# Y-Claw/Multilevel-GNN

Measured on AMD Instinct MI355X. Metric: graphs/sec fwd+bwd, 3-level GNN on 10k-node d=128 synthetic; HBM GB/s %peak, higher is better.
Workload: dtype f32; 1 GPU; configs[1]: ER graphs N=10000 E=160000 x64 per GPU, d=128, 3 GENConv(softmax, res+, LayerNorm) + projection pooling G=25000 k=2 + DiffPool 146->37->10, fp32; step = CSR build (of the next batch, on a second stream) + fwd + bwd + grad all-reduce + Adam; graphs_per_gpu=64, global_batch=64, parallelism=dp1, world_size=1, allreduce_bytes=1429768

## Files before the change

include/mlgnn.h:

```cpp
#ifndef MLGNN_H
#define MLGNN_H

#include <stdint.h>

#ifdef __cplusplus
extern "C" {
#endif

#define MLGNN_ABI_VERSION 19

#define MLGNN_E_NULL      (-1)
#define MLGNN_E_SHAPE     (-2)
#define MLGNN_E_MODE      (-3)
#define MLGNN_E_DTYPE     (-4)
#define MLGNN_E_WORKSPACE (-5)
#define MLGNN_E_ALIGN     (-6)

#define MLGNN_MSG_IDENTITY 0
#define MLGNN_MSG_WEIGHTED 1
#define MLGNN_MSG_GEN      2

#define MLGNN_EDGE_NONE  0
#define MLGNN_EDGE_RANK1 1
#define MLGNN_EDGE_FULL  2
// ... 105 lines not shown
                            float* workspace,
                            int64_t workspace_floats, const uint8_t* keep_mask, float keep_scale,
                            int64_t rows, int64_t d, int relu,
                            int dtype, void* stream);

int64_t mlgnn_linear_wgrad_workspace_floats(int64_t N, int64_t M, int64_t K, int dtype);
int mlgnn_linear_wgrad(const void* grad_out, const void* x, const float* x_gamma, const float* x_beta,
                       const float* grad_out_row_max, const float* x_row_max, float* grad_w_b, float* workspace,
                       int64_t workspace_floats, int64_t N, int64_t M, int64_t K, int dtype,
                       void* stream);

int mlgnn_diffpool_fwd_supported(int64_t N, int64_t K, int64_t C);
int mlgnn_diffpool_fwd(const void* z, const void* adj, const void* s_logits, void* s_out,
                       void* x_out, void* adj_out, float* partial, int64_t B, int64_t N,
                       int64_t K, int64_t C, int adj_batched, int dtype, void* stream);

int mlgnn_diffpool_bwd(const void* z, const void* adj, const void* s_softmax, const void* grad_x,
                       const void* grad_adj_out, const float* coef, void* grad_z, void* grad_s,
                       void* grad_adj, int64_t B, int64_t N, int64_t K, int64_t C,
                       int adj_batched, int dtype, void* stream);

int mlgnn_dense_sage_supported(int64_t n, int64_t C, int64_t O, int need_grad_adj);
int64_t mlgnn_dense_sage_bwd_workspace_floats(int64_t B, int64_t C, int64_t O);
int mlgnn_dense_sage_fwd(const void* x, const void* adj, const void* w_rel, const void* w_root,
                         const float* bias, void* y, float* rinv, int64_t B, int64_t n, int64_t C,
                         int64_t O, int adj_batched, int normalize, int dtype, void* stream);
int mlgnn_dense_sage_bwd(const void* grad_y, const void* y, const float* rinv, const void* x,
                         const void* adj, const void* w_rel, const void* w_root, void* grad_x,
                         void* grad_adj, float* grad_w, float* workspace, int64_t workspace_floats,
                         int64_t B, int64_t n, int64_t C, int64_t O, int adj_batched, int normalize,
                         int dtype, void* stream);

int64_t mlgnn_coo_to_csr_workspace_bytes(int64_t N, int64_t E);
int mlgnn_coo_to_csr(const int64_t* edge_index, int64_t E, int64_t N,
                     int32_t* rowptr, int32_t* col, int32_t* eid,
                     int32_t* rowptr_t, int32_t* col_t, int32_t* pos_t, int32_t* eid_t,
                     int32_t* bad_ids, void* workspace, int64_t workspace_bytes, void* stream);

int mlgnn_edge_table_to_csr(const float* attr, int64_t row_stride, int64_t r, int64_t width,
                            const int32_t* eid, const int32_t* eid_t, float* by_dst, float* by_src,
                            int64_t E, void* stream);

int64_t mlgnn_msgnorm_bwd_workspace_floats(int64_t rows, int64_t d);
int mlgnn_msgnorm_add_fwd(const void* x, const void* m, const float* scale, void* h,
                          int64_t rows, int64_t d, int dtype, void* stream);
int mlgnn_msgnorm_add_bwd(const void* grad_h, const void* x, const void* m, const float* scale,
                          void* grad_x, void* grad_m, float* grad_scale, float* workspace,
                          int64_t workspace_floats, int64_t rows, int64_t d, int dtype, void* stream);

int64_t mlgnn_segment_pool_workspace_bytes(int64_t B, int64_t d);
int mlgnn_segment_pool_fwd(const void* x, const int32_t* ptr, void* out, int32_t* argmax,
                           void* workspace, int64_t workspace_bytes, int64_t B, int64_t d,
                           int kind, int dtype, void* stream);

int mlgnn_tallgemm_supported(int64_t N, int64_t R, int64_t J, int dtype);
int64_t mlgnn_tallgemm_workspace_bytes(int64_t R, int64_t J, int dtype);
int mlgnn_tallgemm_nt(const void* a, const void* bt, int bt_transposed, const float* bias, const void* residual,
                      const float* row_max, int ln_mode, const float* gamma, const float* beta, float ln_eps,
                      float* rstd_out, float* row_max_out, void* c, void* workspace, int64_t workspace_bytes, int64_t N, int64_t R, int64_t J, int dtype, void* stream);

int mlgnn_tallgemm_nt_shift_supported(int64_t N, int64_t R, int64_t J);
int mlgnn_tallgemm_nt_shift(const float* a, const float* bt, int bt_transposed, const float* row_max, const float* lse,
                            const int32_t* rowptr, float* c, float* grad_shifted, int32_t* shift_flag, void* workspace,
                            int64_t workspace_bytes, int64_t N, int64_t R, int64_t J, void* stream);

int mlgnn_tallgemm_bf16_shift_supported(int64_t N, int64_t R, int64_t J);
// ... 232 lines not shown
```

multilevel-gnn_amd/csrc/graph.hip:

```cpp
#include <hipcub/hipcub.hpp>
#include "common.h"
#include "launch.h"
#include "mlgnn.h"

namespace mlgnn {

__device__ __forceinline__ int checked_id(int64_t v, int N, int* bad) {
  if (v < 0 || v >= N) {
    if (bad) atomicAdd(bad, 1);
    return v < 0 ? 0 : N - 1;
  }
  return (int)v;
}

constexpr int kCsrThreads = 1024, kCsrMaxPer = 20;
constexpr int kCsrWindow = 16384;
constexpr int kCsrTargetBlocks = 512;

__device__ __forceinline__ int csr_chunk_of_block() {
  const int nb = gridDim.x, q = nb / kXcds, r = nb % kXcds, xcd = blockIdx.x % kXcds;
  return (xcd < r ? xcd * (q + 1) : r * (q + 1) + (xcd - r) * q) + blockIdx.x / kXcds;
}

__device__ __forceinline__ int block_min(int v, int* slot) {
  if (threadIdx.x == 0) *slot = INT32_MAX;
  __syncthreads();
#pragma unroll
  for (int off = 32; off > 0; off >>= 1) v = min(v, __shfl_xor(v, off));
  if ((threadIdx.x & (kWave - 1)) == 0) atomicMin(slot, v);
  __syncthreads();
  return *slot;
}

__device__ __forceinline__ void csr_count_side(const int64_t* __restrict__ in64, int* __restrict__ out32,
                                               int* __restrict__ cnt, int64_t e0, int64_t n, int per, int N, int* bad,
                                               int* h, int* slot) {
  int k[kCsrMaxPer];
  int mk = INT32_MAX;
  const int64_t first = e0 + threadIdx.x;
  const int64_t left = n - first;
  const int lim = (int)(left < (int64_t)per * kCsrThreads ? (left < 0 ? 0 : left) : (int64_t)per * kCsrThreads);
  const int64_t* __restrict__ in = in64 + first;
  int* __restrict__ out = out32 + first;
#pragma unroll
  for (int g = 0; g < kCsrMaxPer; g += 5) {
    int64_t raw[5];
#pragma unroll
    for (int q = 0; q < 5; ++q) raw[q] = ((g + q) * kCsrThreads < lim) ? in[(g + q) * kCsrThreads] : -1;
#pragma unroll
    for (int q = 0; q < 5; ++q) {
      k[g + q] = -1;
      if ((g + q) * kCsrThreads < lim) {
        k[g + q] = checked_id(raw[q], N, bad);
        out[(g + q) * kCsrThreads] = k[g + q];
        mk = min(mk, k[g + q]);
      }
    }
    __builtin_amdgcn_sched_barrier(0);
  }
  for (int i = threadIdx.x; i < kCsrWindow / 4; i += kCsrThreads) reinterpret_cast<int4*>(h)[i] = make_int4(0, 0, 0, 0);
  const int base = block_min(mk, slot);
#pragma unroll
  for (int q = 0; q < kCsrMaxPer; ++q) {
    if (q >= per || k[q] < 0) continue;
    const int o = k[q] - base;
    if (o < kCsrWindow) atomicAdd(h + o, 1); else atomicAdd(cnt + k[q], 1);
  }
  __syncthreads();
  for (int i = threadIdx.x; i < kCsrWindow; i += kCsrThreads)
    if (h[i]) atomicAdd(cnt + base + i, h[i]);
  __syncthreads();
}

__global__ __launch_bounds__(kCsrThreads, 8) void csr_count_kernel(const int64_t* __restrict__ src64,
                                                                   const int64_t* __restrict__ dst64,
                                                                   int* __restrict__ src32, int* __restrict__ dst32,
                                                                   int* __restrict__ cnt_dst, int* __restrict__ cnt_src,
                                                                   int64_t n, int per, int N, int* bad) {
  __shared__ __attribute__((aligned(16))) int h[kCsrWindow];
  __shared__ int slot;
  const int64_t e0 = (int64_t)csr_chunk_of_block() * per * kCsrThreads;
  csr_count_side(dst64, dst32, cnt_dst, e0, n, per, N, bad, h, &slot);
  csr_count_side(src64, src32, cnt_src, e0, n, per, N, bad, h, &slot);
}

__global__ __launch_bounds__(kCsrThreads, 8) void csr_place_kernel(const int* __restrict__ key,
                                                                   const int* __restrict__ rowptr,
                                                                   int* __restrict__ cursor, int* __restrict__ out,
                                                                   int64_t n, int per) {
  __shared__ __attribute__((aligned(16))) int h[kCsrWindow];
  __shared__ int slot;
  const int64_t e0 = (int64_t)csr_chunk_of_block() * per * kCsrThreads;
  int k[kCsrMaxPer];
  int mk = INT32_MAX;
#pragma unroll
  for (int q = 0; q < kCsrMaxPer; ++q) {
    const int64_t i = e0 + threadIdx.x + (int64_t)q * kCsrThreads;
    k[q] = (q < per && i < n) ? key[i] : -1;
    if (k[q] >= 0) mk = min(mk, k[q]);
  }
  for (int i = threadIdx.x; i < kCsrWindow / 4; i += kCsrThreads) reinterpret_cast<int4*>(h)[i] = make_int4(0, 0, 0, 0);
  const int base = block_min(mk, &slot);
#pragma unroll
  for (int q = 0; q < kCsrMaxPer; ++q)
    if (q < per && k[q] >= 0 && k[q] - base < kCsrWindow) atomicAdd(h + (k[q] - base), 1);
  __syncthreads();
  for (int i = threadIdx.x; i < kCsrWindow; i += kCsrThreads) {
    const int c = h[i];
    if (c) h[i] = rowptr[base + i] + atomicAdd(cursor + base + i, c);
  }
  __syncthreads();
#pragma unroll
  for (int q = 0; q < kCsrMaxPer; ++q) {
    if (q >= per || k[q] < 0) continue;
    const int64_t i = e0 + threadIdx.x + (int64_t)q * kCsrThreads;
    const int o = k[q] - base;
    const int where = o < kCsrWindow ? atomicAdd(h + o, 1) : rowptr[k[q]] + atomicAdd(cursor + k[q], 1);
    out[where] = (int)i;
  }
}

template <int WIDTH>
__device__ __forceinline__ int wave_sort(int v, int lane) {
#pragma unroll
  for (int k = 2; k <= WIDTH; k <<= 1) {
    int p = lane ^ (k - 1);
    int o = __shfl(v, p);
    v = (lane < p) ? min(v, o) : max(v, o);
#pragma unroll
    for (int j = k >> 2; j >= 1; j >>= 1) {
      p = lane ^ j;
      o = __shfl(v, p);
      v = (lane < p) ? min(v, o) : max(v, o);
    }
  }
  return v;
}

struct RowOut { const int* src32; int* col; int* rowkey; const int* eid; int* col_t; int* eid_t; };

template <bool BY_SRC>
__device__ __forceinline__ void emit(const RowOut& o, int slot, int v, int row) {
  if constexpr (!BY_SRC) { o.col[slot] = o.src32[v]; o.rowkey[slot] = row; }
  else { o.col_t[slot] = o.rowkey[v]; o.eid_t[slot] = o.eid[v]; }
}

constexpr int kSortPairs = 4;
constexpr int kSortRows = 2 * kSortPairs;

template <bool BY_SRC>
__global__ __launch_bounds__(kBlock) void csr_sort_rows_kernel(const int* __restrict__ rowptr, int* __restrict__ data,
                                                               int N, int* __restrict__ long_rows,
                                                               int* __restrict__ long_count, const RowOut o) {
  const int lane = threadIdx.x & (kWave - 1);
  const int r0 = (blockIdx.x * kWavesPerBlock + threadIdx.x / kWave) * kSortRows;
  if (r0 >= N) return;
  const int rp = rowptr[min(r0 + min(lane, kSortRows), N)];
  const int deg_l = __shfl_down(rp, 1) - rp;
  const bool small = __builtin_amdgcn_ballot_w64(lane < kSortRows && deg_l > 32) == 0;
  if (small) {
    const int half = lane >> 5, l = lane & 31;
    int v[kSortPairs], beg[kSortPairs], dg[kSortPairs];
#pragma unroll
    for (int p = 0; p < kSortPairs; ++p) {
      beg[p] = __shfl(rp, 2 * p + half);
      dg[p] = __shfl(rp, 2 * p + half + 1) - beg[p];
      v[p] = l < dg[p] ? data[beg[p] + l] : INT32_MAX;
    }
#pragma unroll
    for (int p = 0; p < kSortPairs; ++p) v[p] = wave_sort<32>(v[p], lane);
    int g0[kSortPairs], g1[kSortPairs];
#pragma unroll
    for (int p = 0; p < kSortPairs; ++p) {
      g0[p] = 0; g1[p] = 0;
      if (l < dg[p]) {
        if constexpr (!BY_SRC) g0[p] = o.src32[v[p]];
        else { g0[p] = o.rowkey[v[p]]; g1[p] = o.eid[v[p]]; }
      }
    }
#pragma unroll
    for (int p = 0; p < kSortPairs; ++p) {
      if (l >= dg[p]) continue;
      const int slot = beg[p] + l;
      data[slot] = v[p];
      if constexpr (!BY_SRC) { o.col[slot] = g0[p]; o.rowkey[slot] = r0 + 2 * p + half; }
      else { o.col_t[slot] = g0[p]; o.eid_t[slot] = g1[p]; }
    }
    return;
  }
  for (int w = 0; w < kSortRows && r0 + w < N; ++w) {
    const int beg = __shfl(rp, w), deg = __shfl(rp, w + 1) - beg;
    if (deg <= kWave) {
      int v = lane < deg ? data[beg + lane] : INT32_MAX;
      v = wave_sort<kWave>(v, lane);
      if (lane < deg) { data[beg + lane] = v; emit<BY_SRC>(o, beg + lane, v, r0 + w); }
    } else if (lane == 0) {
      long_rows[atomicAdd(long_count, 1)] = r0 + w;
    }
  }
}

constexpr int kLongLds = 4096;
template <bool BY_SRC>
__global__ __launch_bounds__(kBlock) void csr_sort_long_rows_kernel(const int* __restrict__ rowptr,
                                                                    int* __restrict__ data,
                                                                    const int* __restrict__ long_rows,
                                                                    const int* __restrict__ long_count,
                                                                    const RowOut o) {
  __shared__ int buf[kLongLds];
  const int count = *long_count;
  for (int it = blockIdx.x; it < count; it += gridDim.x) {
    const int r = long_rows[it];
    const int beg = rowptr[r], n = rowptr[r + 1] - beg;
    int P = 1;
    while (P < n) P <<= 1;
    const bool in_lds = n <= kLongLds;
    int* a = in_lds ? buf : data + beg;
    if (in_lds) {
      for (int i = threadIdx.x; i < n; i += kBlock) buf[i] = data[beg + i];
    }
    __syncthreads();
    for (int k = 2; k <= P; k <<= 1) {
      for (int i = threadIdx.x; i < P / 2; i += kBlock) {
        const int blk = i / (k / 2), off = i % (k / 2);
        const int x = blk * k + off, y = blk * k + k - 1 - off;
        if (y < n) { const int u = a[x], w = a[y]; if (u > w) { a[x] = w; a[y] = u; } }
      }
      __syncthreads();
      for (int j = k >> 2; j >= 1; j >>= 1) {
        for (int i = threadIdx.x; i < P / 2; i += kBlock) {
          const int x = (i / j) * 2 * j + i % j, y = x + j;
// ... 16 lines not shown
                                  float* __restrict__ by_dst, float* __restrict__ by_src, int64_t n) {
  const int64_t i = (int64_t)blockIdx.x * blockDim.x + threadIdx.x;
  if (i >= n) return;
  const float* a = attr + (int64_t)eid[i] * stride;
  const float* b = attr + (int64_t)eid_t[i] * stride;
  for (int k = 0; k < width; ++k) {
    by_dst[i * width + k] = k < r ? a[k] : 0.f;
    by_src[i * width + k] = k < r ? b[k] : 0.f;
  }
}

__global__ __launch_bounds__(256) void edge_table_w1_kernel(const float* __restrict__ attr, int64_t stride,
                                                            const int4* __restrict__ eid, const int4* __restrict__ eid_t,
                                                            float4* __restrict__ by_dst, float4* __restrict__ by_src,
                                                            int64_t n4) {
  const int64_t i = (int64_t)blockIdx.x * blockDim.x + threadIdx.x;
  if (i >= n4) return;
  const int4 e = eid[i], t = eid_t[i];
  float4 a, b;
  a.x = attr[(int64_t)e.x * stride]; a.y = attr[(int64_t)e.y * stride];
  a.z = attr[(int64_t)e.z * stride]; a.w = attr[(int64_t)e.w * stride];
  b.x = attr[(int64_t)t.x * stride]; b.y = attr[(int64_t)t.y * stride];
  b.z = attr[(int64_t)t.z * stride]; b.w = attr[(int64_t)t.w * stride];
  by_dst[i] = a;
  by_src[i] = b;
}

static size_t scan_temp_bytes(int64_t n) {
  size_t bytes = 0;
  (void)hipcub::DeviceScan::ExclusiveSum(nullptr, bytes, (const int*)nullptr, (int*)nullptr, (int)n, (hipStream_t)0);
  return bytes;
}

struct CsrWs {
  int *src32, *dst32, *rowkey, *cnt_dst, *cnt_src, *cur_dst, *cur_src, *long_rows, *long_rows_t, *long_count;
  size_t zero_bytes;
  void* scan_temp; size_t scan_bytes; size_t total;
};
static CsrWs csr_ws(void* workspace, int64_t N, int64_t E) {
  CsrWs w;
  const size_t e4 = align256((size_t)E * 4), n4 = align256((size_t)(N + 1) * 4);
  char* p = (char*)(((uintptr_t)workspace + 255) & ~(uintptr_t)255);
  w.src32 = (int*)p; p += e4;
  w.dst32 = (int*)p; p += e4;
  w.rowkey = (int*)p; p += e4;
  w.long_rows = (int*)p; p += n4;
  w.long_rows_t = (int*)p; p += n4;
  w.cnt_dst = (int*)p; p += n4;
  w.cnt_src = (int*)p; p += n4;
  w.cur_dst = (int*)p; p += n4;
  w.cur_src = (int*)p; p += n4;
  w.long_count = (int*)p; p += 256;
  w.zero_bytes = (size_t)(p - (char*)w.cnt_dst);
  w.scan_bytes = scan_temp_bytes(N + 1);
  w.scan_temp = p; p += align256(w.scan_bytes);
  w.total = (size_t)(p - (char*)(((uintptr_t)workspace + 255) & ~(uintptr_t)255)) + 256;
  return w;
}

static int csr_per_thread(int64_t E) {
  const int64_t target = (E + kCsrTargetBlocks - 1) / kCsrTargetBlocks;
  const int64_t per = (target + kCsrThreads - 1) / kCsrThreads;
  return (int)(per < 1 ? 1 : per > kCsrMaxPer ? kCsrMaxPer : per);
}

}

using namespace mlgnn;

extern "C" int64_t mlgnn_coo_to_csr_workspace_bytes(int64_t N, int64_t E) {
  if (N < 0 || E < 0 || N > INT32_MAX - 1 || E > INT32_MAX) return MLGNN_E_SHAPE;
  return (int64_t)csr_ws(nullptr, N, E).total;
}

extern "C" int mlgnn_coo_to_csr(const int64_t* edge_index, int64_t E, int64_t N,
                                int32_t* rowptr, int32_t* col, int32_t* eid,
                                int32_t* rowptr_t, int32_t* col_t, int32_t* pos_t, int32_t* eid_t,
                                int32_t* bad_ids, void* workspace, int64_t workspace_bytes, void* stream) {
  if (N < 0 || E < 0 || N > INT32_MAX - 1 || E > INT32_MAX) return MLGNN_E_SHAPE;
  if (!rowptr || !rowptr_t) return MLGNN_E_NULL;
  hipStream_t s = (hipStream_t)stream;
  if (bad_ids) (void)hipMemsetAsync(bad_ids, 0, 4, s);
  if (E == 0) {
    (void)hipMemsetAsync(rowptr, 0, (size_t)(N + 1) * 4, s);
    (void)hipMemsetAsync(rowptr_t, 0, (size_t)(N + 1) * 4, s);
    return (int)hipGetLastError();
  }
  if (!edge_index || !col || !eid || !col_t || !pos_t || !eid_t || !workspace) return MLGNN_E_NULL;
  if (N == 0) return MLGNN_E_SHAPE;
  const CsrWs w = csr_ws(workspace, N, E);
  if (workspace_bytes < (int64_t)w.total) return MLGNN_E_WORKSPACE;
  const int per = csr_per_thread(E);
  const int64_t chunk = (int64_t)per * kCsrThreads;
  const unsigned gC = (unsigned)((E + chunk - 1) / chunk);
  const unsigned gRows = (unsigned)(((N + kSortRows - 1) / kSortRows + kWavesPerBlock - 1) / kWavesPerBlock);
  hipError_t err;

  (void)hipMemsetAsync(w.cnt_dst, 0, w.zero_bytes, s);
  hipLaunchKernelGGL(csr_count_kernel, dim3(gC), dim3(kCsrThreads), 0, s, edge_index, edge_index + E, w.src32,
                     w.dst32, w.cnt_dst, w.cnt_src, E, per, (int)N, bad_ids);
  size_t sb = w.scan_bytes;
  err = hipcub::DeviceScan::ExclusiveSum(w.scan_temp, sb, w.cnt_dst, rowptr, (int)(N + 1), s);
  if (err != hipSuccess) return (int)err;
  err = hipcub::DeviceScan::ExclusiveSum(w.scan_temp, sb, w.cnt_src, rowptr_t, (int)(N + 1), s);
  if (err != hipSuccess) return (int)err;

  RowOut o;
  o.src32 = w.src32; o.col = col; o.rowkey = w.rowkey; o.eid = eid; o.col_t = col_t; o.eid_t = eid_t;
  hipLaunchKernelGGL(csr_place_kernel, dim3(gC), dim3(kCsrThreads), 0, s, w.dst32, rowptr, w.cur_dst, eid, E, per);
  hipLaunchKernelGGL(csr_sort_rows_kernel<false>, dim3(gRows), dim3(kBlock), 0, s, rowptr, eid, (int)N, w.long_rows,
                     w.long_count, o);
  hipLaunchKernelGGL(csr_sort_long_rows_kernel<false>, dim3(256), dim3(kBlock), 0, s, rowptr, eid, w.long_rows,
                     w.long_count, o);

  hipLaunchKernelGGL(csr_place_kernel, dim3(gC), dim3(kCsrThreads), 0, s, col, rowptr_t, w.cur_src, pos_t, E, per);
  hipLaunchKernelGGL(csr_sort_rows_kernel<true>, dim3(gRows), dim3(kBlock), 0, s, rowptr_t, pos_t, (int)N, w.long_rows_t,
                     w.long_count + 1, o);
  hipLaunchKernelGGL(csr_sort_long_rows_kernel<true>, dim3(256), dim3(kBlock), 0, s, rowptr_t, pos_t, w.long_rows_t,
                     w.long_count + 1, o);
  return (int)hipGetLastError();
}

namespace mlgnn {
__global__ __launch_bounds__(256) void sage_rewrite_kernel(const int64_t* __restrict__ src, const int64_t* __restrict__ dst,
                                                          const float* __restrict__ attr, int64_t attr_stride,
                                                          int64_t* __restrict__ out_src, int64_t* __restrict__ out_dst,
                                                          float* __restrict__ out_w, int64_t E, int64_t N) {
  const int64_t stride = (int64_t)gridDim.x * blockDim.x;
  for (int64_t i = (int64_t)blockIdx.x * blockDim.x + threadIdx.x; i < E + N; i += stride) {
    if (i < E) {
      const int64_t a = src[i], b = dst[i];
      const bool loop = a == b;
      out_src[i] = loop ? N : a;
      out_dst[i] = loop ? N : b;
      if (out_w) out_w[i] = attr ? attr[i * attr_stride] : 1.f;
    } else {
      out_src[i] = i - E;
      out_dst[i] = i - E;
      if (out_w) out_w[i] = 1.f;
    }
  }
}
}

extern "C" int mlgnn_sage_rewrite(const int64_t* edge_index, const float* edge_attr, int64_t attr_stride, int64_t E,
                                  int64_t N, int64_t* out_edge_index, float* out_weight, void* stream) {
  if (N < 0 || E < 0 || N > INT32_MAX - 2 || E + N > INT32_MAX || (edge_attr && attr_stride < 1)) return MLGNN_E_SHAPE;
  if (E + N == 0) return 0;
  if ((E > 0 && !edge_index) || !out_edge_index) return MLGNN_E_NULL;
  const int64_t n = E + N;
// ... 76 lines not shown
```

multilevel-gnn_amd/mlgnn/_lib.py:

```python
import ctypes
import os

LIB = os.environ.get("MLGNN_LIB") or os.path.join(os.path.dirname(os.path.abspath(__file__)), "libmlgnn.so")

_c = ctypes
_P = _c.c_void_p
_I64 = _c.c_int64
_INT = _c.c_int
_F = _c.c_float

SIGNATURES = {
    "mlgnn_version": (_INT, []),
    "mlgnn_csr_aggregate_bwd_workspace_floats": (_I64, [_I64, _I64, _INT, _INT, _INT, _INT]),
    "mlgnn_csr_aggregate_fwd": (_INT, [_P, _P, _P, _P, _P, _P, _P, _P, _P, _P, _P, _P, _P,
                                       _I64, _I64, _INT, _INT, _INT, _INT, _INT, _F, _F, _P, _P, _F, _INT, _P, _P]),
    "mlgnn_csr_aggregate_bwd": (_INT, [_P, _P, _P, _P, _P, _P, _P, _P, _P, _P, _P, _P, _P, _P, _P,
                                       _P, _P, _P, _P, _I64,
                                       _I64, _I64, _INT, _INT, _INT, _INT, _INT, _INT, _F, _F, _P, _P, _F, _INT, _INT, _P,
                                       _P, _P, _P]),
    "mlgnn_csr_aggregate_bwd_ln_workspace_floats": (_I64, [_I64, _I64]),
    "mlgnn_csr_aggregate_bwd_ln": (_INT, [_P, _P, _P, _P, _P, _P, _P, _P, _P, _P, _P, _P, _P, _P, _P,
                                          _P, _P, _P, _P, _I64,
                                          _I64, _I64, _INT, _INT, _INT, _INT, _INT, _INT, _F, _F, _P, _P, _F, _INT, _INT, _P,
                                          _P, _P, _P, _P]),
# ... 1 lines not shown
    "mlgnn_power_bwd_prologue": (_INT, [_P, _P, _P, _P, _P, _F, _P, _P, _P, _P, _I64, _I64, _I64, _INT, _P]),
    "mlgnn_embedding_bwd": (_INT, [_P, _P, _P, _P, _I64, _I64, _INT, _P]),
    "mlgnn_max_table_grad_supported": (_INT, [_I64, _I64, _I64]),
    "mlgnn_max_table_grad_workspace_floats": (_I64, [_I64, _I64, _I64]),
    "mlgnn_max_table_grad": (_INT, [_P, _P, _P, _P, _P, _I64, _I64, _I64, _I64, _INT, _P]),
    "mlgnn_max_table_grad_by_type": (_INT, [_P, _P, _P, _P, _P, _P, _P, _P, _I64, _I64, _I64, _INT, _P]),
    "mlgnn_csr_aggregate_bwd_slots_offset_floats": (_I64, [_I64, _I64, _INT]),
    "mlgnn_max_sparse_supported": (_INT, [_I64, _I64]),
    "mlgnn_max_sparse_records": (_I64, [_I64, _I64, _I64]),
    "mlgnn_max_winners": (_INT, [_P, _P, _P, _P, _P, _I64, _I64, _P]),
    "mlgnn_max_sparse_bwd": (_INT, [_P, _P, _P, _P, _P, _P, _I64, _I64, _P]),
    "mlgnn_max_sparse_table_grad": (_INT, [_P, _P, _P, _P, _P, _I64, _I64, _I64, _INT, _P]),
    "mlgnn_table_grad_bytes": (_I64, [_I64, _I64]),
    "mlgnn_table_grad_begin": (_INT, [_P, _I64, _I64, _P, _P]),
    "mlgnn_table_grad_finish": (_INT, [_P, _P, _I64, _I64, _INT, _P]),
    "mlgnn_segment_project_fwd": (_INT, [_P, _P, _P, _P, _P, _P, _I64, _I64, _I64, _I64, _I64, _I64, _INT, _P]),
    "mlgnn_segment_project_bwd": (_INT, [_P, _P, _P, _P, _P, _P, _P, _P, _P, _P, _P,
                                         _I64, _I64, _I64, _I64, _I64, _I64, _I64, _INT, _P]),
    "mlgnn_layernorm_bwd_workspace_floats": (_I64, [_I64, _I64, _INT]),
    "mlgnn_layernorm_act_fwd": (_INT, [_P, _P, _P, _P, _P, _P, _P, _P, _F, _I64, _I64, _F, _INT, _INT, _P]),
    "mlgnn_layernorm_act_bwd": (_INT, [_P, _P, _P, _P, _P, _P, _P, _P, _P, _P, _P, _I64, _P, _F, _I64, _I64, _INT, _INT, _P]),
    "mlgnn_linear_wgrad_workspace_floats": (_I64, [_I64, _I64, _I64, _INT]),
    "mlgnn_tallgemm_bf16_shift_supported": (_INT, [_I64, _I64, _I64]),
    "mlgnn_tallgemm_bf16_shift": (_INT, [_P, _P, _P, _P, _P, _P, _P, _I64, _I64, _I64, _I64, _P]),
    "mlgnn_linear_bwd_supported": (_INT, [_I64, _I64, _I64, _INT]),
    "mlgnn_linear_bwd_workspace_floats": (_I64, [_I64, _I64, _I64, _INT]),
    "mlgnn_linear_bwd": (_INT, [_P, _P, _P, _P, _INT, _P, _INT, _P, _P, _P, _P, _P, _P, _P, _P, _P, _P, _I64,
                                _I64, _I64, _I64, _P]),
    "mlgnn_linear_wgrad": (_INT, [_P, _P, _P, _P, _P, _P, _P, _P, _I64, _I64, _I64, _I64, _INT, _P]),
    "mlgnn_diffpool_fwd_supported": (_INT, [_I64, _I64, _I64]),
    "mlgnn_diffpool_fwd": (_INT, [_P, _P, _P, _P, _P, _P, _P, _I64, _I64, _I64, _I64, _INT, _INT, _P]),
    "mlgnn_coo_to_csr_workspace_bytes": (_I64, [_I64, _I64]),
    "mlgnn_coo_to_csr": (_INT, [_P, _I64, _I64, _P, _P, _P, _P, _P, _P, _P, _P, _P, _I64, _P]),
    "mlgnn_msgnorm_bwd_workspace_floats": (_I64, [_I64, _I64]),
    "mlgnn_msgnorm_add_fwd": (_INT, [_P, _P, _P, _P, _I64, _I64, _INT, _P]),
    "mlgnn_msgnorm_add_bwd": (_INT, [_P, _P, _P, _P, _P, _P, _P, _P, _I64, _I64, _I64, _INT, _P]),
    "mlgnn_diffpool_bwd": (_INT, [_P, _P, _P, _P, _P, _P, _P, _P, _P, _I64, _I64, _I64, _I64, _INT, _INT, _P]),
    "mlgnn_edge_table_to_csr": (_INT, [_P, _I64, _I64, _I64, _P, _P, _P, _P, _I64, _P]),
    "mlgnn_dense_sage_supported": (_INT, [_I64, _I64, _I64, _INT]),
    "mlgnn_dense_sage_bwd_workspace_floats": (_I64, [_I64, _I64, _I64]),
    "mlgnn_dense_sage_fwd": (_INT, [_P, _P, _P, _P, _P, _P, _P, _I64, _I64, _I64, _I64, _INT, _INT, _INT, _P]),
    "mlgnn_dense_sage_bwd": (_INT, [_P, _P, _P, _P, _P, _P, _P, _P, _P, _P, _P, _I64,
                                    _I64, _I64, _I64, _I64, _INT, _INT, _INT, _P]),
    "mlgnn_segment_pool_workspace_bytes": (_I64, [_I64, _I64]),
    "mlgnn_segment_pool_fwd": (_INT, [_P, _P, _P, _P, _P, _I64, _I64, _I64, _INT, _INT, _P]),
    "mlgnn_tallgemm_supported": (_INT, [_I64, _I64, _I64, _INT]),
    "mlgnn_tallgemm_workspace_bytes": (_I64, [_I64, _I64, _INT]),
    "mlgnn_tallgemm_nt": (_INT, [_P, _P, _INT, _P, _P, _P, _INT, _P, _P, _F, _P, _P, _P, _P, _I64, _I64, _I64, _I64, _INT, _P]),
    "mlgnn_tallgemm_nt_shift_supported": (_INT, [_I64, _I64, _I64]),
    "mlgnn_tallgemm_nt_shift": (_INT, [_P, _P, _INT, _P, _P, _P, _P, _P, _P, _P, _I64, _I64, _I64, _I64, _P]),
    "mlgnn_tallgemm_lnin_postln_supported": (_INT, [_I64, _I64, _I64]),
    "mlgnn_tallgemm_lnin_postln": (_INT, [_P, _P, _P, _P, _P, _P, _P, _P, _P, _F, _INT, _P, _P, _P, _P, _P, _I64,
                                          _I64, _I64, _I64, _P]),
    "mlgnn_tallgemm_lnbwd_supported": (_INT, [_I64, _I64, _I64]),
    "mlgnn_tallgemm_lnbwd_workspace_bytes": (_I64, [_I64, _I64]),
    "mlgnn_tallgemm_lnbwd": (_INT, [_P, _P, _INT, _P, _P, _P, _P, _P, _P, _P, _P, _P, _I64, _I64, _I64, _I64, _P]),
    "mlgnn_csr_replicate": (_INT, [_P] * 14 + [_I64, _I64, _I64, _P]),
    "mlgnn_sage_rewrite": (_INT, [_P, _P, _I64, _I64, _I64, _P, _P, _P]),
    "mlgnn_tallgemm_dual_supported": (_INT, [_I64, _I64, _I64, _I64]),
    "mlgnn_tallgemm_dual": (_INT, [_P, _P, _P, _P, _F, _P, _P, _P, _P, _P, _I64, _I64, _I64, _I64, _I64, _P]),
    "mlgnn_transpose_batched": (_INT, [_P, _P, _I64, _I64, _I64, _P]),
    "mlgnn_sage_fold_fwd": (_INT, [_P, _P, _P, _P, _P, _I64, _I64, _INT, _P]),
    "mlgnn_sage_fold_bwd": (_INT, [_P, _P, _P, _P, _P, _P, _I64, _I64, _INT, _P]),
    "mlgnn_leaky_relu_bwd": (_INT, [_P, _P, _P, _F, _P, _P, _I64, _I64, _P]),
    "mlgnn_node_embed_fwd": (_INT, [_P, _P, _P, _P, _I64, _I64, _I64, _P]),
    "mlgnn_node_embed_bwd": (_INT, [_P, _P, _P, _I64, _I64, _I64, _P]),
# ... 165 lines not shown
```

multilevel-gnn_amd/mlgnn/graph.py:

```python
import ctypes
import os

import torch

from . import _lib

HUB_CAP = int(os.environ.get("MLGNN_HUB_CAP", "256"))
SAGE_HUB_CAP = int(os.environ.get("MLGNN_SAGE_HUB_CAP", "64")) if HUB_CAP > 0 else 0
_SHARED_TOPOLOGY = os.environ.get("MLGNN_SHARED_TOPOLOGY", "1") == "1"


class CSRGraph:

    def __init__(self, edge_index, num_nodes):
        if edge_index.dim() != 2 or edge_index.shape[0] != 2:
            raise ValueError("edge_index must be [2, E]")
        N = int(num_nodes)
        E = int(edge_index.shape[1])
        if N >= 2 ** 31 or E >= 2 ** 31:
            raise ValueError("int32 index range exceeded")
        dev = edge_index.device
        self.num_nodes, self.num_edges, self.device = N, E, dev
        if edge_index.is_cuda:
            self._build_device(edge_index)
# ... 109 lines not shown
            if tabs[6] is not False:
                return False
        return True

    def hub_arg(self, direction, d):
        tabs = self.hub_tables(direction)
        if tabs is None:
            return None, ()
        if tabs[6] is None and tabs[5].query():
            tabs[6] = int(tabs[4][0]) > 0
        if tabs[6] is False:
            return None, ()
        vrows, hubs, counts, cap_rows = tabs[:4]
        nbytes = int(_lib.lib.mlgnn_hub_scratch_bytes(cap_rows, d))
        tmp = torch.empty(nbytes, dtype=torch.uint8, device=self.device)
        st = _lib.HubStruct(getattr(self, "hub_cap", HUB_CAP), cap_rows, vrows.data_ptr(), hubs.data_ptr(), counts.data_ptr(), tmp.data_ptr(), nbytes)
        return ctypes.byref(st), (st, tmp)

    def _build_device(self, edge_index):
        N, E, dev = self.num_nodes, self.num_edges, self.device
        ei = edge_index.to(torch.int64).contiguous()
        i32 = dict(dtype=torch.int32, device=dev)
        self.rowptr, self.rowptr_t = torch.empty(N + 1, **i32), torch.empty(N + 1, **i32)
        self.col, self.eid = torch.empty(E, **i32), torch.empty(E, **i32)
        self.col_t, self.pos_t, self.eid_t = torch.empty(E, **i32), torch.empty(E, **i32), torch.empty(E, **i32)
        nbytes = int(_lib.lib.mlgnn_coo_to_csr_workspace_bytes(N, E))
        ws = torch.empty(max(nbytes, 1), dtype=torch.uint8, device=dev)
        self._bad_ids = torch.empty(1, **i32)
        rc = _lib.lib.mlgnn_coo_to_csr(ei.data_ptr(), E, N, self.rowptr.data_ptr(), _lib.ptr(self.col),
                                       _lib.ptr(self.eid), self.rowptr_t.data_ptr(), _lib.ptr(self.col_t),
                                       _lib.ptr(self.pos_t), _lib.ptr(self.eid_t), self._bad_ids.data_ptr(),
                                       ws.data_ptr(), nbytes, torch.cuda.current_stream().cuda_stream)
        _lib.check(rc, "mlgnn_coo_to_csr")

    def validate(self):
        bad = getattr(self, "_bad_ids", None)
        if bad is not None and int(bad.item()) != 0:
            raise ValueError("%d edge endpoints outside [0, %d)" % (int(bad.item()), self.num_nodes))
        return self

    def _build_host(self, edge_index):
        N = self.num_nodes
        src, dst = edge_index[0].long(), edge_index[1].long()
        if edge_index.numel() and (int(edge_index.min()) < 0 or int(edge_index.max()) >= N):
            raise ValueError("edge endpoints outside [0, %d)" % N)
        order = torch.sort(dst, stable=True).indices
        col = src[order]
        order_t = torch.sort(col, stable=True).indices
        self.rowptr = self._ptr(dst, N)
        self.col = col.to(torch.int32)
        self.eid = order.to(torch.int32)
        self.rowptr_t = self._ptr(src, N)
        self.col_t = dst[order][order_t].to(torch.int32)
        self.pos_t = order_t.to(torch.int32)
        self.eid_t = order[order_t].to(torch.int32)

    def to(self, device):
        for name in ("rowptr", "col", "eid", "rowptr_t", "col_t", "pos_t", "eid_t"):
            setattr(self, name, getattr(self, name).to(device))
        self.device = torch.device(device)
        self._deg, self._scalar_cache, self._table_cache, self._hub = None, None, None, {}
        return self

    @staticmethod
    def _ptr(index, N):
        counts = torch.bincount(index, minlength=N)
# ... 207 lines not shown
```

Measured before the change: 5553 graphs/s.

## Add row-block LDS bucketing path for CSR construction with legacy fallback

```diff
diff --git a/include/mlgnn.h b/include/mlgnn.h
--- a/include/mlgnn.h
+++ b/include/mlgnn.h
@@ -161,6 +161,7 @@
                          int dtype, void* stream);
 
 int64_t mlgnn_coo_to_csr_workspace_bytes(int64_t N, int64_t E);
+int64_t mlgnn_coo_to_csr_flags_offset(int64_t N, int64_t E);
 int mlgnn_coo_to_csr(const int64_t* edge_index, int64_t E, int64_t N,
                      int32_t* rowptr, int32_t* col, int32_t* eid,
                      int32_t* rowptr_t, int32_t* col_t, int32_t* pos_t, int32_t* eid_t,
diff --git a/multilevel-gnn_amd/csrc/csr_rowblock.h b/multilevel-gnn_amd/csrc/csr_rowblock.h
--- /dev/null
+++ b/multilevel-gnn_amd/csrc/csr_rowblock.h
@@ -0,0 +1,33 @@
+#pragma once
+#include <cstdint>
+
+namespace mlgnn {
+
+constexpr int kRowblockCap = 16384;
+constexpr int kRowblockFill = kRowblockCap / 4 * 3;
+constexpr int kRowblockMinRows = 128, kRowblockMaxRows = 1024;
+constexpr int kRowblockLdsBudget = 80 * 1024;
+
+struct RowblockShape {
+  int rows;
+  int64_t blocks;
+  int lds_bytes;
+};
+
+inline int rowblock_lds_bytes(int rows) {
+  return ((2 * rows + 1 + kRowblockCap) * 4 + 15) & ~15;
+}
+
+inline RowblockShape rowblock_shape(int64_t N, int64_t E) {
+  int64_t r = E > 0 ? (int64_t)kRowblockFill * (N > 0 ? N : 0) / E : kRowblockMaxRows;
+  r = r / 8 * 8;
+  if (r < kRowblockMinRows) r = kRowblockMinRows;
+  if (r > kRowblockMaxRows) r = kRowblockMaxRows;
+  RowblockShape s;
+  s.rows = (int)r;
+  s.blocks = N > 0 ? (N + r - 1) / r : 0;
+  s.lds_bytes = rowblock_lds_bytes(s.rows);
+  return s;
+}
+
+}
diff --git a/multilevel-gnn_amd/csrc/graph.hip b/multilevel-gnn_amd/csrc/graph.hip
--- a/multilevel-gnn_amd/csrc/graph.hip
+++ b/multilevel-gnn_amd/csrc/graph.hip
@@ -1,6 +1,7 @@
 #include <hipcub/hipcub.hpp>
 #include "common.h"
 #include "launch.h"
+#include "csr_rowblock.h"
 #include "mlgnn.h"
 
 namespace mlgnn {
@@ -32,11 +33,24 @@
   return *slot;
 }
 
+__device__ __forceinline__ int block_min_max(int lo, int hi, int* slot) {
+  if (threadIdx.x == 0) { slot[0] = INT32_MAX; slot[1] = INT32_MIN; }
+  __syncthreads();
+#pragma unroll
+  for (int off = 32; off > 0; off >>= 1) {
+    lo = min(lo, __shfl_xor(lo, off));
+    hi = max(hi, __shfl_xor(hi, off));
+  }
+  if ((threadIdx.x & (kWave - 1)) == 0) { atomicMin(slot, lo); atomicMax(slot + 1, hi); }
+  __syncthreads();
+  return slot[0];
+}
+
 __device__ __forceinline__ void csr_count_side(const int64_t* __restrict__ in64, int* __restrict__ out32,
                                                int* __restrict__ cnt, int64_t e0, int64_t n, int per, int N, int* bad,
-                                               int* h, int* slot) {
+                                               int* h, int* slot, int* __restrict__ interval) {
   int k[kCsrMaxPer];
-  int mk = INT32_MAX;
+  int mk = INT32_MAX, xk = INT32_MIN;
   const int64_t first = e0 + threadIdx.x;
   const int64_t left = n - first;
   const int lim = (int)(left < (int64_t)per * kCsrThreads ? (left < 0 ? 0 : left) : (int64_t)per * kCsrThreads);
@@ -54,12 +68,14 @@
         k[g + q] = checked_id(raw[q], N, bad);
         out[(g + q) * kCsrThreads] = k[g + q];
         mk = min(mk, k[g + q]);
+        xk = max(xk, k[g + q]);
       }
     }
     __builtin_amdgcn_sched_barrier(0);
   }
   for (int i = threadIdx.x; i < kCsrWindow / 4; i += kCsrThreads) reinterpret_cast<int4*>(h)[i] = make_int4(0, 0, 0, 0);
-  const int base = block_min(mk, slot);
+  const int base = block_min_max(mk, xk, slot);
+  if (threadIdx.x == 0) { interval[0] = base; interval[1] = slot[1]; }
 #pragma unroll
   for (int q = 0; q < kCsrMaxPer; ++q) {
     if (q >= per || k[q] < 0) continue;
@@ -76,20 +92,27 @@
                                                                    const int64_t* __restrict__ dst64,
                                                                    int* __restrict__ src32, int* __restrict__ dst32,
                                                                    int* __restrict__ cnt_dst, int* __restrict__ cnt_src,
-                                                                   int64_t n, int per, int N, int* bad) {
+                                                                   int64_t n, int per, int N, int* bad,
+                                                                   int* __restrict__ chunk_tab,
+                                                                   int* __restrict__ flags, int legacy) {
   __shared__ __attribute__((aligned(16))) int h[kCsrWindow];
-  __shared__ int slot;
-  const int64_t e0 = (int64_t)csr_chunk_of_block() * per * kCsrThreads;
-  csr_count_side(dst64, dst32, cnt_dst, e0, n, per, N, bad, h, &slot);
-  csr_count_side(src64, src32, cnt_src, e0, n, per, N, bad, h, &slot);
+  __shared__ int slot[2];
+  const int chunk = csr_chunk_of_block();
+  const int64_t e0 = (int64_t)chunk * per * kCsrThreads;
+  if (legacy && blockIdx.x == 0 && threadIdx.x == 0) { flags[0] = 1; flags[1] = 1; }
+  csr_count_side(dst64, dst32, cnt_dst, e0, n, per, N, bad, h, slot, chunk_tab + 4 * (int64_t)chunk);
+  csr_count_side(src64, src32, cnt_src, e0, n, per, N, bad, h, slot, chunk_tab + 4 * (int64_t)chunk + 2);
 }
 
 __global__ __launch_bounds__(kCsrThreads, 8) void csr_place_kernel(const int* __restrict__ key,
                                                                    const int* __restrict__ rowptr,
                                                                    int* __restrict__ cursor, int* __restrict__ out,
-                                                                   int64_t n, int per) {
+                                                                   int64_t n, int per, const int* __restrict__ flag,
+                                                                   int* __restrict__ long_count) {
   __shared__ __attribute__((aligned(16))) int h[kCsrWindow];
   __shared__ int slot;
+  if (*flag == 0) return;
+  if (blockIdx.x == 0 && threadIdx.x == 0) *long_count = 0;
   const int64_t e0 = (int64_t)csr_chunk_of_block() * per * kCsrThreads;
   int k[kCsrMaxPer];
   int mk = INT32_MAX;
@@ -151,7 +174,9 @@
 template <bool BY_SRC>
 __global__ __launch_bounds__(kBlock) void csr_sort_rows_kernel(const int* __restrict__ rowptr, int* __restrict__ data,
                                                                int N, int* __restrict__ long_rows,
-                                                               int* __restrict__ long_count, const RowOut o) {
+                                                               int* __restrict__ long_count, const RowOut o,
+                                                               const int* __restrict__ flag) {
+  if (*flag == 0) return;
   const int lane = threadIdx.x & (kWave - 1);
   const int r0 = (blockIdx.x * kWavesPerBlock + threadIdx.x / kWave) * kSortRows;
   if (r0 >= N) return;
@@ -197,6 +222,189 @@
     } else if (lane == 0) {
       long_rows[atomicAdd(long_count, 1)] = r0 + w;
     }
+  }
+}
+
+constexpr int kRowblockMaxSegs = 64;
+constexpr int kRowblockStream = 64;
+constexpr int kRowblockLoads = 4;
+constexpr int64_t kRowblockMaxTable = 65536;
+
+__device__ __forceinline__ int4 load_keys4(const int* __restrict__ key, int64_t i, int n) {
+  if (i + 4 <= n) return *reinterpret_cast<const int4*>(key + i);
+  int4 v;
+  v.x = i < n ? key[i] : -1; v.y = i + 1 < n ? key[i + 1] : -1;
+  v.z = i + 2 < n ? key[i + 2] : -1; v.w = i + 3 < n ? key[i + 3] : -1;
+  return v;
+}
+
+__device__ __forceinline__ int slot_value(int v, int n) { return (int)min((unsigned)v, (unsigned)n - 1u); }
+
+template <bool BY_SRC>
+__global__ __launch_bounds__(kCsrThreads, 8) void csr_rowblock_kernel(
+    const int* __restrict__ key,
+    const int* __restrict__ rowptr,
+    const int* __restrict__ seg_tab,
+    const int* __restrict__ seg_ptr,
+    int nseg, int seg_len,
+    int* __restrict__ data,
+    int N, int n, int R, int* __restrict__ blk_tab, int* __restrict__ long_rows, int* __restrict__ long_count,
+    int* __restrict__ flags, const RowOut o) {
+  extern __shared__ __attribute__((aligned(16))) int rb_lds[];
+  __shared__ int seg_beg[kRowblockMaxSegs], seg_end[kRowblockMaxSegs];
+  __shared__ int stop, nkept, lo_s, hi_s;
+  __shared__ unsigned total;
+  int* rp = rb_lds;
+  int* cur = rb_lds + R + 1;
+  int* bucket = cur + R;
+  const int tid = threadIdx.x;
+  const int b = csr_chunk_of_block();
+  const int r0 = b * R, nrows = min(R, N - r0), r1 = r0 + nrows;
+  if (tid == 0) {
+    stop = flags[BY_SRC] | flags[0];
+    nkept = 0; total = 0u; lo_s = INT32_MAX; hi_s = -1;
+  }
+  for (int i = tid; i <= nrows; i += kCsrThreads) rp[i] = rowptr[r0 + i];
+  for (int i = tid; i < nrows; i += kCsrThreads) cur[i] = 0;
+  __syncthreads();
+  if (stop) {
+    if (BY_SRC && tid == 0) flags[1] = 1;
+    return;
+  }
+  const int base = rp[0], cnt = rp[nrows] - base;
+  if (cnt > kRowblockCap) {
+    if (tid == 0) flags[BY_SRC] = 1;
+    return;
+  }
+  if (cnt == 0) {
+    if (!BY_SRC && tid == 0) { blk_tab[2 * b] = INT32_MAX; blk_tab[2 * b + 1] = -1; }
+    return;
+  }
+  for (int i = tid; i < nseg; i += kCsrThreads) {
+    int sb, se, klo, khi;
+    if constexpr (!BY_SRC) {
+      const int4 t = reinterpret_cast<const int4*>(seg_tab)[i];
+      const int64_t first = (int64_t)i * seg_len;
+      klo = t.x; khi = t.y;
+      sb = (int)first;
+      se = (int)min(first + seg_len, (int64_t)n);
+    } else {
+      klo = seg_tab[2 * i]; khi = seg_tab[2 * i + 1];
+      sb = seg_ptr[min((int64_t)i * seg_len, (int64_t)N)];
+      se = seg_ptr[min((int64_t)(i + 1) * seg_len, (int64_t)N)];
+    }
+    if (sb < se && klo < r1 && khi >= r0) {
+      const int k = atomicAdd(&nkept, 1);
+      if (k < kRowblockMaxSegs) { seg_beg[k] = sb; seg_end[k] = se; }
+      atomicAdd(&total, (unsigned)(se - sb));
+    }
+  }
+  __syncthreads();
+  const int ns = nkept;
+  if (ns > kRowblockMaxSegs || total > (unsigned)kRowblockStream * (unsigned)max(cnt, kRowblockFill)) {
+    if (tid == 0) flags[BY_SRC] = 1;
+    return;
+  }
+  for (int s = 0; s < ns; ++s) {
+    const int sb = seg_beg[s], se = seg_end[s];
+    for (int64_t i0 = (int64_t)(sb & ~3) + 4 * tid; i0 < se; i0 += 4 * kCsrThreads * kRowblockLoads) {
+      int4 v[kRowblockLoads];
+#pragma unroll
+      for (int u = 0; u < kRowblockLoads; ++u) {
+        const int64_t i = i0 + (int64_t)u * 4 * kCsrThreads;
+        v[u] = i < se ? load_keys4(key, i, n) : make_int4(-1, -1, -1, -1);
+      }
+#pragma unroll
+      for (int u = 0; u < kRowblockLoads; ++u) {
+        const int64_t i = i0 + (int64_t)u * 4 * kCsrThreads;
+        const int kk[4] = {v[u].x, v[u].y, v[u].z, v[u].w};
+#pragma unroll
+        for (int j = 0; j < 4; ++j) {
+          const unsigned row = (unsigned)(kk[j] - r0);
+          if (row < (unsigned)nrows && i + j >= sb && i + j < se) {
+            const int where = rp[row] - base + atomicAdd(cur + row, 1);
+            if ((unsigned)where < (unsigned)cnt) bucket[where] = (int)(i + j);
+          }
+        }
+      }
+    }
+  }
+  __syncthreads();
+  const int lane = tid & (kWave - 1);
+  int lo = INT32_MAX, hi = -1;
+  for (int g = (tid / kWave) * kSortRows; g < nrows; g += (kCsrThreads / kWave) * kSortRows) {
+    const int rpl = rp[min(g + min(lane, kSortRows), nrows)];
+    const int deg_l = __shfl_down(rpl, 1) - rpl;
+    const bool small = __builtin_amdgcn_ballot_w64(lane < kSortRows && deg_l > 32) == 0;
+    if (small) {
+      const int half = lane >> 5, l = lane & 31;
+      int v[kSortPairs], beg[kSortPairs], dg[kSortPairs];
+#pragma unroll
+      for (int p = 0; p < kSortPairs; ++p) {
+        beg[p] = __shfl(rpl, 2 * p + half);
+        dg[p] = __shfl(rpl, 2 * p + half + 1) - beg[p];
+        v[p] = l < dg[p] ? slot_value(bucket[beg[p] - base + l], n) : INT32_MAX;
+      }
+#pragma unroll
+      for (int p = 0; p < kSortPairs; ++p) v[p] = wave_sort<32>(v[p], lane);
+      int g0[kSortPairs], g1[kSortPairs];
+#pragma unroll
+      for (int p = 0; p < kSortPairs; ++p) {
+        g0[p] = 0; g1[p] = 0;
+        if (l < dg[p]) {
+          if constexpr (!BY_SRC) g0[p] = o.src32[v[p]];
+          else { g0[p] = o.rowkey[v[p]]; g1[p] = o.eid[v[p]]; }
+        }
+      }
+#pragma unroll
+      for (int p = 0; p < kSortPairs; ++p) {
+        if (l >= dg[p]) continue;
+        const int slot = beg[p] + l;
+        data[slot] = v[p];
+        if constexpr (!BY_SRC) {
+          o.col[slot] = g0[p]; o.rowkey[slot] = r0 + g + 2 * p + half;
+          lo = min(lo, g0[p]); hi = max(hi, g0[p]);
+        } else { o.col_t[slot] = g0[p]; o.eid_t[slot] = g1[p]; }
+      }
+      continue;
+    }
+#pragma unroll 1
+    for (int w = 0; w < kSortRows && g + w < nrows; ++w) {
+      const int beg = __shfl(rpl, w), deg = __shfl(rpl, w + 1) - beg;
+      if (deg <= kWave) {
+        int v = lane < deg ? slot_value(bucket[beg - base + lane], n) : INT32_MAX;
+        v = wave_sort<kWave>(v, lane);
+        if (lane < deg) {
+          data[beg + lane] = v;
+          if constexpr (!BY_SRC) {
+            const int c = o.src32[v];
+            o.col[beg + lane] = c; o.rowkey[beg + lane] = r0 + g + w;
+            lo = min(lo, c); hi = max(hi, c);
+          } else { o.col_t[beg + lane] = o.rowkey[v]; o.eid_t[beg + lane] = o.eid[v]; }
+        }
+      } else {
+#pragma unroll 1
+        for (int i = lane; i < deg; i += kWave) {
+          const int v = slot_value(bucket[beg - base + i], n);
+          data[beg + i] = v;
+          if constexpr (!BY_SRC) {
+            const int c = o.src32[v];
+            lo = min(lo, c); hi = max(hi, c);
+          }
+        }
+        if (lane == 0) long_rows[atomicAdd(long_count, 1)] = r0 + g + w;
+      }
+    }
+  }
+  if constexpr (!BY_SRC) {
+#pragma unroll
+    for (int off = 32; off > 0; off >>= 1) {
+      lo = min(lo, __shfl_xor(lo, off));
+      hi = max(hi, __shfl_xor(hi, off));
+    }
+    if (lane == 0) { atomicMin(&lo_s, lo); atomicMax(&hi_s, hi); }
+    __syncthreads();
+    if (tid == 0) { blk_tab[2 * b] = lo_s; blk_tab[2 * b + 1] = hi_s; }
   }
 }
 
@@ -279,8 +487,17 @@
   return bytes;
 }
 
+static int csr_per_thread(int64_t E) {
+  const int64_t target = (E + kCsrTargetBlocks - 1) / kCsrTargetBlocks;
+  const int64_t per = (target + kCsrThreads - 1) / kCsrThreads;
+  return (int)(per < 1 ? 1 : per > kCsrMaxPer ? kCsrMaxPer : per);
+}
+
 struct CsrWs {
   int *src32, *dst32, *rowkey, *cnt_dst, *cnt_src, *cur_dst, *cur_src, *long_rows, *long_rows_t, *long_count;
+  int *chunk_tab, *blk_tab;
+  int* flags;
+  int64_t chunks; RowblockShape rb;
   size_t zero_bytes;
   void* scan_temp; size_t scan_bytes; size_t total;
 };
@@ -293,11 +510,17 @@
   w.rowkey = (int*)p; p += e4;
   w.long_rows = (int*)p; p += n4;
   w.long_rows_t = (int*)p; p += n4;
+  const int64_t chunk = (int64_t)csr_per_thread(E) * kCsrThreads;
+  w.chunks = (E + chunk - 1) / chunk;
+  w.rb = rowblock_shape(N, E);
+  w.chunk_tab = (int*)p; p += align256((size_t)w.chunks * 16);
+  w.blk_tab = (int*)p; p += align256((size_t)w.rb.blocks * 8);
   w.cnt_dst = (int*)p; p += n4;
   w.cnt_src = (int*)p; p += n4;
   w.cur_dst = (int*)p; p += n4;
   w.cur_src = (int*)p; p += n4;
   w.long_count = (int*)p; p += 256;
+  w.flags = w.long_count + 2;
   w.zero_bytes = (size_t)(p - (char*)w.cnt_dst);
   w.scan_bytes = scan_temp_bytes(N + 1);
   w.scan_temp = p; p += align256(w.scan_bytes);
@@ -305,12 +528,6 @@
   return w;
 }
 
-static int csr_per_thread(int64_t E) {
-  const int64_t target = (E + kCsrTargetBlocks - 1) / kCsrTargetBlocks;
-  const int64_t per = (target + kCsrThreads - 1) / kCsrThreads;
-  return (int)(per < 1 ? 1 : per > kCsrMaxPer ? kCsrMaxPer : per);
-}
-
 }
 
 using namespace mlgnn;
@@ -318,6 +535,12 @@
 extern "C" int64_t mlgnn_coo_to_csr_workspace_bytes(int64_t N, int64_t E) {
   if (N < 0 || E < 0 || N > INT32_MAX - 1 || E > INT32_MAX) return MLGNN_E_SHAPE;
   return (int64_t)csr_ws(nullptr, N, E).total;
+}
+
+extern "C" int64_t mlgnn_coo_to_csr_flags_offset(int64_t N, int64_t E) {
+  if (N < 0 || E < 0 || N > INT32_MAX - 1 || E > INT32_MAX) return MLGNN_E_SHAPE;
+  const CsrWs w = csr_ws(nullptr, N, E);
+  return (int64_t)((char*)w.flags - (char*)nullptr);
 }
 
 extern "C" int mlgnn_coo_to_csr(const int64_t* edge_index, int64_t E, int64_t N,
@@ -339,13 +562,24 @@
   if (workspace_bytes < (int64_t)w.total) return MLGNN_E_WORKSPACE;
   const int per = csr_per_thread(E);
   const int64_t chunk = (int64_t)per * kCsrThreads;
-  const unsigned gC = (unsigned)((E + chunk - 1) / chunk);
+  const unsigned gC = (unsigned)w.chunks;
   const unsigned gRows = (unsigned)(((N + kSortRows - 1) / kSortRows + kWavesPerBlock - 1) / kWavesPerBlock);
   hipError_t err;
 
   (void)hipMemsetAsync(w.cnt_dst, 0, w.zero_bytes, s);
+  static const bool rowblock_on = [] { const char* e = getenv("MLGNN_CSR_ROWBLOCK"); return !(e && e[0] == '0'); }();
+  const bool rowblock = rowblock_on && w.chunks <= kRowblockMaxTable && w.rb.blocks <= kRowblockMaxTable && aligned(col);
+  const unsigned gB = (unsigned)w.rb.blocks;
+  if (rowblock) {
+    static const hipError_t lds_ok = [] {
+      const int most = rowblock_lds_bytes(kRowblockMaxRows);
+      const hipError_t e = allow_dynamic_lds(csr_rowblock_kernel<false>, most);
+      return e != hipSuccess ? e : allow_dynamic_lds(csr_rowblock_kernel<true>, most);
+    }();
+    if (lds_ok != hipSuccess) return (int)lds_ok;
+  }
   hipLaunchKernelGGL(csr_count_kernel, dim3(gC), dim3(kCsrThreads), 0, s, edge_index, edge_index + E, w.src32,
-                     w.dst32, w.cnt_dst, w.cnt_src, E, per, (int)N, bad_ids);
+                     w.dst32, w.cnt_dst, w.cnt_src, E, per, (int)N, bad_ids, w.chunk_tab, w.flags, rowblock ? 0 : 1);
   size_t sb = w.scan_bytes;
   err = hipcub::DeviceScan::ExclusiveSum(w.scan_temp, sb, w.cnt_dst, rowptr, (int)(N + 1), s);
   if (err != hipSuccess) return (int)err;
@@ -354,15 +588,25 @@
 
   RowOut o;
   o.src32 = w.src32; o.col = col; o.rowkey = w.rowkey; o.eid = eid; o.col_t = col_t; o.eid_t = eid_t;
-  hipLaunchKernelGGL(csr_place_kernel, dim3(gC), dim3(kCsrThreads), 0, s, w.dst32, rowptr, w.cur_dst, eid, E, per);
+  if (rowblock)
+    hipLaunchKernelGGL(csr_rowblock_kernel<false>, dim3(gB), dim3(kCsrThreads), w.rb.lds_bytes, s, w.dst32, rowptr,
+                       w.chunk_tab, (const int*)nullptr, (int)w.chunks, (int)chunk, eid, (int)N, (int)E, w.rb.rows,
+                       w.blk_tab, w.long_rows, w.long_count, w.flags, o);
+  hipLaunchKernelGGL(csr_place_kernel, dim3(gC), dim3(kCsrThreads), 0, s, w.dst32, rowptr, w.cur_dst, eid, E, per,
+                     w.flags, w.long_count);
   hipLaunchKernelGGL(csr_sort_rows_kernel<false>, dim3(gRows), dim3(kBlock), 0, s, rowptr, eid, (int)N, w.long_rows,
-                     w.long_count, o);
+                     w.long_count, o, w.flags);
   hipLaunchKernelGGL(csr_sort_long_rows_kernel<false>, dim3(256), dim3(kBlock), 0, s, rowptr, eid, w.long_rows,
                      w.long_count, o);
 
-  hipLaunchKernelGGL(csr_place_kernel, dim3(gC), dim3(kCsrThreads), 0, s, col, rowptr_t, w.cur_src, pos_t, E, per);
+  if (rowblock)
+    hipLaunchKernelGGL(csr_rowblock_kernel<true>, dim3(gB), dim3(kCsrThreads), w.rb.lds_bytes, s, col, rowptr_t,
+                       w.blk_tab, rowptr, (int)w.rb.blocks, w.rb.rows, pos_t, (int)N, (int)E, w.rb.rows,
+                       (int*)nullptr, w.long_rows_t, w.long_count + 1, w.flags, o);
+  hipLaunchKernelGGL(csr_place_kernel, dim3(gC), dim3(kCsrThreads), 0, s, col, rowptr_t, w.cur_src, pos_t, E, per,
+                     w.flags + 1, w.long_count + 1);
   hipLaunchKernelGGL(csr_sort_rows_kernel<true>, dim3(gRows), dim3(kBlock), 0, s, rowptr_t, pos_t, (int)N, w.long_rows_t,
-                     w.long_count + 1, o);
+                     w.long_count + 1, o, w.flags + 1);
   hipLaunchKernelGGL(csr_sort_long_rows_kernel<true>, dim3(256), dim3(kBlock), 0, s, rowptr_t, pos_t, w.long_rows_t,
                      w.long_count + 1, o);
   return (int)hipGetLastError();
diff --git a/multilevel-gnn_amd/mlgnn/_lib.py b/multilevel-gnn_amd/mlgnn/_lib.py
--- a/multilevel-gnn_amd/mlgnn/_lib.py
+++ b/multilevel-gnn_amd/mlgnn/_lib.py
@@ -57,6 +57,7 @@
     "mlgnn_diffpool_fwd": (_INT, [_P, _P, _P, _P, _P, _P, _P, _I64, _I64, _I64, _I64, _INT, _INT, _P]),
     "mlgnn_coo_to_csr_workspace_bytes": (_I64, [_I64, _I64]),
     "mlgnn_coo_to_csr": (_INT, [_P, _I64, _I64, _P, _P, _P, _P, _P, _P, _P, _P, _P, _I64, _P]),
+    "mlgnn_coo_to_csr_flags_offset": (_I64, [_I64, _I64]),
     "mlgnn_msgnorm_bwd_workspace_floats": (_I64, [_I64, _I64]),
     "mlgnn_msgnorm_add_fwd": (_INT, [_P, _P, _P, _P, _I64, _I64, _INT, _P]),
     "mlgnn_msgnorm_add_bwd": (_INT, [_P, _P, _P, _P, _P, _P, _P, _P, _I64, _I64, _I64, _INT, _P]),
diff --git a/multilevel-gnn_amd/mlgnn/graph.py b/multilevel-gnn_amd/mlgnn/graph.py
--- a/multilevel-gnn_amd/mlgnn/graph.py
+++ b/multilevel-gnn_amd/mlgnn/graph.py
@@ -165,6 +165,9 @@
                                        _lib.ptr(self.pos_t), _lib.ptr(self.eid_t), self._bad_ids.data_ptr(),
                                        ws.data_ptr(), nbytes, torch.cuda.current_stream().cuda_stream)
         _lib.check(rc, "mlgnn_coo_to_csr")
+        if E > 0:
+            off = (-ws.data_ptr()) % 256 + int(_lib.lib.mlgnn_coo_to_csr_flags_offset(N, E))
+            self._legacy_path = ws[off:off + 8].view(torch.int32).clone()
 
     def validate(self):
         bad = getattr(self, "_bad_ids", None)
```

Result: no change. 5580 graphs/s, median of 6 (+0.5%).
